# ShannonAI/GNN-LM

Hardware: AMD Instinct MI355X
Metric: eval tokens/sec on WikiText-103 (k=1024, GNN+KNN); test ppl match (higher is better)
Workload: dtype f32

## Files before the change

gnn-lm_amd/csrc/gemm_f32.hip:

```cpp
#include "kernels.h"

namespace gnnlm {

typedef float f32x16 __attribute__((ext_vector_type(16)));
typedef __bf16 bf16x8 __attribute__((ext_vector_type(8)));
typedef _Float16 f16x8 __attribute__((ext_vector_type(8)));

namespace {
constexpr int BK = 32, LDS_LD = BK + 4;
#ifndef GNNLM_GEMM_NBUF
#define GNNLM_GEMM_NBUF 1
#endif
constexpr int NBUF = GNNLM_GEMM_NBUF;
enum { EPI_STORE = 0, EPI_LSE = 1 };

__device__ __forceinline__ unsigned bf16_rn(float x) {
    const unsigned u = __float_as_uint(x);
    return (u + 0x7FFFu + ((u >> 16) & 1u)) >> 16;
}
__device__ __forceinline__ float bf16_to_f32(unsigned h) { return __uint_as_float(h << 16); }

template <int BM, int BN, int EPI, int NS>
__global__ __launch_bounds__(256, 3) void gemm_nt_f32_kernel(const GemmParams p) {
    constexpr int TM = BM / 64, TN = BN / 64;
    constexpr int LA = BM / 32, LW = BN / 32;
    constexpr int STAGE = (BM + BN) * LDS_LD;
    constexpr int SPLIT_LD = 20;
    constexpr int PLANE = (BM + BN) * SPLIT_LD;
    constexpr int LDS_FLOATS = NS == 0 ? NBUF * STAGE : NS * PLANE;
    __shared__ __attribute__((aligned(16))) float lds[LDS_FLOATS];

    const int tid = threadIdx.x, lane = tid & 63, wave = tid >> 6;
    const int wm = wave >> 1, wn = wave & 1;
    const int half = lane >> 5, l32 = lane & 31;

    int M = p.M;
    if (p.m_dev) M = min(M, *p.m_dev);
    if (p.m_out && blockIdx.x == 0 && threadIdx.x == 0) *p.m_out = M;
    const int tiles_n = (p.N + BN - 1) / BN;
    const int tiles_m = ((p.m_dev ? M : p.M) + BM - 1) / BM;
    const unsigned n_tiles = (unsigned)(tiles_m * tiles_n);
    const unsigned n_work = n_tiles * (unsigned)(p.batch1 * p.batch2);
    unsigned v = blockIdx.x;
    if (v >= n_work) return;

    const int kq = (tid & 7) * 4;
    const int srow = tid >> 3;
    const float* ap[LA];
    const float* wp[LW];
    float4 ra[LA], rw[LW];
    const int nk_full = p.K / BK;
    const bool k_tail = (p.K % BK) != 0;
    const float4 z4 = make_float4(0.f, 0.f, 0.f, 0.f);
    int m0x, n0x, b1x, b2x;

#define GNNLM_TILE_SETUP(w_)                                                                 \
    {                                                                                        \
        const unsigned by_ = (w_) / n_tiles, t = (w_) - by_ * n_tiles;                       \
        b1x = by_ / p.batch2; b2x = by_ % p.batch2;                                          \
        int tm, tn;                                                                          \
        if (p.tile_order == 1) { tm = t / tiles_n; tn = t % tiles_n; }                       \
        else if (p.tile_order == 2) { tn = t / tiles_m; tm = t % tiles_m; }                  \
        else {                   \
            const int GM = p.tile_order - 2;                                                 \
            const int band = t / (GM * tiles_n);                                             \
            const int m_in = min(GM, tiles_m - band * GM);                                   \
            const int r = t - band * GM * tiles_n;                                           \
            tn = r / m_in;                                                                   \
            tm = band * GM + r % m_in;                                                       \
        }                                                                                    \
        m0x = tm * BM; n0x = tn * BN;                                                        \
        const float* A_ = p.A + b1x * p.sA1 + b2x * p.sA2;                                   \
        const float* W_ = p.W + b1x * p.sW1 + b2x * p.sW2;                                   \
        _Pragma("unroll") for (int i = 0; i < LA; ++i) {                                     \
            const int gr = m0x + srow + 32 * i;                                              \
            int64_t ar = gr < M ? (p.a_rows ? (int64_t)p.a_rows[gr] : (int64_t)gr) : 0;      \
            if (ar < 0) ar = 0;       \
            ap[i] = A_ + ar * p.lda;                                                         \
        }                                                                                    \
        _Pragma("unroll") for (int i = 0; i < LW; ++i) {                                     \
            const int gn = n0x + srow + 32 * i;                                              \
            wp[i] = W_ + (int64_t)(gn < p.N ? gn : 0) * p.ldw;                               \
        }                                                                                    \
    }

#define GNNLM_LOAD_TILE(kt)                                                                  \
    {                                                                                        \
        const int k_ = (kt) * BK + kq;                                                       \
        _Pragma("unroll") for (int i_ = 0; i_ < LA; ++i_)                                    \
            ra[i_] = *reinterpret_cast<const float4*>(ap[i_] + k_);                          \
        _Pragma("unroll") for (int i_ = 0; i_ < LW; ++i_)                                    \
            rw[i_] = *reinterpret_cast<const float4*>(wp[i_] + k_);                          \
    }
#define GNNLM_LOAD_TILE_GUARDED(kt)                                                          \
    {                                                                                        \
        int k_ = (kt) * BK + kq;                                                             \
        const bool kin_ = k_ < p.K;                                                          \
        k_ = kin_ ? k_ : 0;                                                                  \
        _Pragma("unroll") for (int i_ = 0; i_ < LA; ++i_) {                                  \
            ra[i_] = *reinterpret_cast<const float4*>(ap[i_] + k_);                          \
            if (!kin_) ra[i_] = z4;                                                          \
        }                                                                                    \
        _Pragma("unroll") for (int i_ = 0; i_ < LW; ++i_) {                                  \
            rw[i_] = *reinterpret_cast<const float4*>(wp[i_] + k_);                          \
            if (!kin_) rw[i_] = z4;                                                          \
        }                                                                                    \
    }
#define GNNLM_PK_TRUNC(lo_, hi_) ((__float_as_uint(hi_) & 0xFFFF0000u) | (__float_as_uint(lo_) >> 16))
#define GNNLM_SPLIT_STORE(v_, row_)                                                          \
    {                                                                                        \
        char* dst_ = reinterpret_cast<char*>(lds) + (row_) * (SPLIT_LD * 4) + kq * 2;        \
        float r0_ = (v_).x, r1_ = (v_).y, r2_ = (v_).z, r3_ = (v_).w;                        \
        if constexpr (NS == 1) {                                                             \
            typedef _Float16 f16x4_ __attribute__((ext_vector_type(4)));                     \
            *reinterpret_cast<f16x4_*>(dst_) = f16x4_{(_Float16)r0_, (_Float16)r1_, (_Float16)r2_, (_Float16)r3_}; \
        } else if constexpr (NS == 3) {                                                             \
            _Pragma("unroll") for (int pl_ = 0; pl_ < 3; ++pl_) {                            \
                *reinterpret_cast<uint2*>(dst_ + pl_ * (PLANE * 4)) =                        \
                    make_uint2(GNNLM_PK_TRUNC(r0_, r1_), GNNLM_PK_TRUNC(r2_, r3_));          \
                r0_ -= __uint_as_float(__float_as_uint(r0_) & 0xFFFF0000u);                  \
                r1_ -= __uint_as_float(__float_as_uint(r1_) & 0xFFFF0000u);                  \
                r2_ -= __uint_as_float(__float_as_uint(r2_) & 0xFFFF0000u);                  \
                r3_ -= __uint_as_float(__float_as_uint(r3_) & 0xFFFF0000u);                  \
            }                                                                                \
        } else {                                                                             \
            _Pragma("unroll") for (int pl_ = 0; pl_ < 2; ++pl_) {                            \
                const unsigned b0_ = bf16_rn(r0_), b1_ = bf16_rn(r1_), b2_ = bf16_rn(r2_), b3_ = bf16_rn(r3_); \
                *reinterpret_cast<uint2*>(dst_ + pl_ * (PLANE * 4)) = make_uint2(b0_ | (b1_ << 16), b2_ | (b3_ << 16)); \
                r0_ -= __uint_as_float(b0_ << 16);                                           \
                r1_ -= __uint_as_float(b1_ << 16);                                           \
                r2_ -= __uint_as_float(b2_ << 16);                                           \
                r3_ -= __uint_as_float(b3_ << 16);                                           \
            }                                                                                \
        }                                                                                    \
    }
#define GNNLM_STORE_TILE(buf)                                                                \
    if constexpr (NS == 0) {                                                                 \
        float* a_ = &lds[(buf) * STAGE + srow * LDS_LD + kq];                                \
        float* w_ = a_ + BM * LDS_LD;                                                        \
        _Pragma("unroll") for (int i_ = 0; i_ < LA; ++i_)                                    \
            *reinterpret_cast<float4*>(a_ + 32 * i_ * LDS_LD) = ra[i_];                      \
        _Pragma("unroll") for (int i_ = 0; i_ < LW; ++i_)                                    \
            *reinterpret_cast<float4*>(w_ + 32 * i_ * LDS_LD) = rw[i_];                      \
    } else {                                                                                 \
        _Pragma("unroll") for (int i_ = 0; i_ < LA; ++i_) GNNLM_SPLIT_STORE(ra[i_], srow + 32 * i_)        \
        _Pragma("unroll") for (int i_ = 0; i_ < LW; ++i_) GNNLM_SPLIT_STORE(rw[i_], BM + srow + 32 * i_)   \
    }
#define GNNLM_SPLIT_MFMA(PA, PB)                                                             \
    _Pragma("unroll") for (int i = 0; i < TM; ++i)                                           \
        _Pragma("unroll") for (int j = 0; j < TN; ++j)                                       \
            acc[i][j] = EPI == EPI_LSE ? __builtin_amdgcn_mfma_f32_32x32x16_bf16(fb[PB][j], fa[PA][i], acc[i][j], 0, 0, 0)  \
                                       : __builtin_amdgcn_mfma_f32_32x32x16_bf16(fa[PA][i], fb[PB][j], acc[i][j], 0, 0, 0);
#define GNNLM_COMPUTE(buf)                                                                   \
    if constexpr (NS == 1) {                                                                 \
        const char* base_ = reinterpret_cast<const char*>(lds);                              \
        _Pragma("unroll") for (int ks_ = 0; ks_ < BK / 16; ++ks_) {                          \
            f16x8 ha[TM], hb[TN];                                                            \
            _Pragma("unroll") for (int i = 0; i < TM; ++i)                                   \
                ha[i] = *reinterpret_cast<const f16x8*>(base_ + (wm * (BM / 2) + 32 * i + l32) * SPLIT_LD * 4 + 32 * ks_ + 16 * half); \
            _Pragma("unroll") for (int j = 0; j < TN; ++j)                                   \
                hb[j] = *reinterpret_cast<const f16x8*>(base_ + (BM + wn * (BN / 2) + 32 * j + l32) * SPLIT_LD * 4 + 32 * ks_ + 16 * half); \
            _Pragma("unroll") for (int i = 0; i < TM; ++i)                                   \
                _Pragma("unroll") for (int j = 0; j < TN; ++j)                               \
                    acc[i][j] = EPI == EPI_LSE ? __builtin_amdgcn_mfma_f32_32x32x16_f16(hb[j], ha[i], acc[i][j], 0, 0, 0)  \
                                               : __builtin_amdgcn_mfma_f32_32x32x16_f16(ha[i], hb[j], acc[i][j], 0, 0, 0); \
        }                                                                                    \
    } else if constexpr (NS != 0) {                                                                 \
        const char* base_ = reinterpret_cast<const char*>(lds);                              \
        _Pragma("unroll") for (int ks_ = 0; ks_ < BK / 16; ++ks_) {                          \
            bf16x8 fa[NS][TM], fb[NS][TN];                                                   \
            _Pragma("unroll") for (int pl_ = 0; pl_ < NS; ++pl_) {                           \
                _Pragma("unroll") for (int i = 0; i < TM; ++i)                               \
                    fa[pl_][i] = *reinterpret_cast<const bf16x8*>(base_ + (pl_ * (BM + BN) + wm * (BM / 2) + 32 * i + l32) * SPLIT_LD * 4 + 32 * ks_ + 16 * half); \
                _Pragma("unroll") for (int j = 0; j < TN; ++j)                               \
                    fb[pl_][j] = *reinterpret_cast<const bf16x8*>(base_ + (pl_ * (BM + BN) + BM + wn * (BN / 2) + 32 * j + l32) * SPLIT_LD * 4 + 32 * ks_ + 16 * half); \
            }                                                                                \
            if constexpr (NS == 3) { GNNLM_SPLIT_MFMA(2, 0) GNNLM_SPLIT_MFMA(1, 1) GNNLM_SPLIT_MFMA(0, 2) }   \
            GNNLM_SPLIT_MFMA(1, 0) GNNLM_SPLIT_MFMA(0, 1) GNNLM_SPLIT_MFMA(0, 0)             \
        }                                                                                    \
    } else {                                                                                 \
        const float* a_base = &lds[(buf) * STAGE + (wm * (BM / 2) + l32) * LDS_LD + 4 * half];            \
        const float* w_base = &lds[(buf) * STAGE + (BM + wn * (BN / 2) + l32) * LDS_LD + 4 * half];       \
        _Pragma("unroll") for (int s_ = 0; s_ < BK / 8; ++s_) {                              \
            float4 a[TM], b[TN];                                                             \
            _Pragma("unroll") for (int i = 0; i < TM; ++i)                                   \
                a[i] = *reinterpret_cast<const float4*>(a_base + 32 * i * LDS_LD + 8 * s_);  \
            _Pragma("unroll") for (int j = 0; j < TN; ++j)                                   \
                b[j] = *reinterpret_cast<const float4*>(w_base + 32 * j * LDS_LD + 8 * s_);  \
            _Pragma("unroll") for (int i = 0; i < TM; ++i)                                   \
                _Pragma("unroll") for (int j = 0; j < TN; ++j) {                             \
                     \
                    if constexpr (EPI == EPI_LSE) {                                          \
                        acc[i][j] = __builtin_amdgcn_mfma_f32_32x32x2f32(b[j].x, a[i].x, acc[i][j], 0, 0, 0); \
                        acc[i][j] = __builtin_amdgcn_mfma_f32_32x32x2f32(b[j].y, a[i].y, acc[i][j], 0, 0, 0); \
                        acc[i][j] = __builtin_amdgcn_mfma_f32_32x32x2f32(b[j].z, a[i].z, acc[i][j], 0, 0, 0); \
                        acc[i][j] = __builtin_amdgcn_mfma_f32_32x32x2f32(b[j].w, a[i].w, acc[i][j], 0, 0, 0); \
                    } else {                                                                 \
                        acc[i][j] = __builtin_amdgcn_mfma_f32_32x32x2f32(a[i].x, b[j].x, acc[i][j], 0, 0, 0); \
                        acc[i][j] = __builtin_amdgcn_mfma_f32_32x32x2f32(a[i].y, b[j].y, acc[i][j], 0, 0, 0); \
                        acc[i][j] = __builtin_amdgcn_mfma_f32_32x32x2f32(a[i].z, b[j].z, acc[i][j], 0, 0, 0); \
                        acc[i][j] = __builtin_amdgcn_mfma_f32_32x32x2f32(a[i].w, b[j].w, acc[i][j], 0, 0, 0); \
                    }                                                                        \
                }                                                                            \
        }                                                                                    \
    }

#define GNNLM_LOAD_FIRST()                                                                   \
    if (nk_full > 0) GNNLM_LOAD_TILE(0) else GNNLM_LOAD_TILE_GUARDED(0)

    GNNLM_TILE_SETUP(xcd_remap(v, n_work))
    GNNLM_LOAD_FIRST()
    for (;;) {
        const int m0 = m0x, n0 = n0x, b1 = b1x, b2 = b2x;
        f32x16 acc[TM][TN];
#pragma unroll
        for (int i = 0; i < TM; ++i)
#pragma unroll
            for (int j = 0; j < TN; ++j)
#pragma unroll
                for (int r = 0; r < 16; ++r) acc[i][j][r] = 0.f;

        GNNLM_STORE_TILE(0);
        __syncthreads();
        if (nk_full > 0) {
            for (int kt = 0; kt < nk_full; ++kt) {
                constexpr bool ONE_BUF = NBUF == 1 || NS != 0;
                const int buf = ONE_BUF ? 0 : (kt & 1);
                if (kt + 1 < nk_full) GNNLM_LOAD_TILE(kt + 1);
                GNNLM_COMPUTE(buf);
                if (ONE_BUF) __syncthreads();
                if (kt + 1 < nk_full) { GNNLM_STORE_TILE(ONE_BUF ? 0 : (buf ^ 1)); }
                __syncthreads();
            }
            if (k_tail) {
                GNNLM_LOAD_TILE_GUARDED(nk_full);
                GNNLM_STORE_TILE(0);
                __syncthreads();
                GNNLM_COMPUTE(0);
                __syncthreads();
            }
        } else {
            GNNLM_COMPUTE(0);
            __syncthreads();
        }
        v += gridDim.x;
        const bool has_next = v < n_work;
        if (has_next) {
            GNNLM_TILE_SETUP(xcd_remap(v, n_work))
            GNNLM_LOAD_FIRST()
        }
        constexpr int WROWS = BM / 2, WCOLS = BN / 2;
#include "gemm_epilogue.inc"
        __syncthreads();
        if (!has_next) break;
    }
#undef GNNLM_LOAD_FIRST
#undef GNNLM_TILE_SETUP
#undef GNNLM_LOAD_TILE_GUARDED
#undef GNNLM_COMPUTE
#undef GNNLM_SPLIT_MFMA
#undef GNNLM_SPLIT_STORE
#undef GNNLM_PK_TRUNC
#undef GNNLM_LOAD_TILE
#undef GNNLM_STORE_TILE
}

template <int WPR>
__global__ __launch_bounds__(256) void lse_reduce_kernel(const float2* part, int n_parts, int64_t rows,
                                                         const int32_t* m_dev, float* lse) {
    __shared__ float2 red[4];
    const int lane = threadIdx.x & 63, wave = threadIdx.x >> 6;
    const int64_t row = WPR == 1 ? (int64_t)blockIdx.x * 4 + wave : (int64_t)blockIdx.x;
    if (row >= rows || (m_dev && row >= *m_dev)) return;
    const float2* pr = part + row * n_parts;
    const int i0 = WPR == 1 ? lane : threadIdx.x, step = 64 * WPR;
    float m = -INFINITY;
    for (int i = i0; i < n_parts; i += step) m = fmaxf(m, pr[i].x);
    m = wave_max(m);
    if (WPR == 4) {
        if (lane == 0) red[wave].x = m;
        __syncthreads();
        m = fmaxf(fmaxf(red[0].x, red[1].x), fmaxf(red[2].x, red[3].x));
    }
    float s = 0.f;
    for (int i = i0; i < n_parts; i += step) {
        const float2 v = pr[i];
        s += v.x == -INFINITY ? 0.f : v.y * expf(v.x - m);
    }
    s = wave_sum(s);
    if (WPR == 4) {
        if (lane == 0) red[wave].y = s;
        __syncthreads();
        s = (red[0].y + red[1].y) + (red[2].y + red[3].y);
    }
    if (threadIdx.x == (WPR == 1 ? 64 * wave : 0)) lse[row] = m + logf(s);
}

template <int BM, int BN, int NS>
void launch_ns(const GemmParams& p, dim3 grid, hipStream_t stream) {
    if constexpr (BN == 128) {
        if (p.lse_part) {
            hipLaunchKernelGGL((gemm_nt_f32_kernel<BM, BN, EPI_LSE, NS>), grid, dim3(256), 0, stream, p);
            return;
        }
    }
    hipLaunchKernelGGL((gemm_nt_f32_kernel<BM, BN, EPI_STORE, NS>), grid, dim3(256), 0, stream, p);
}
template <int BM, int BN>
void launch(const GemmParams& p, dim3 grid, hipStream_t stream) {
    if (p.precision == 1) launch_ns<BM, BN, 2>(p, grid, stream);
    else if (p.precision == 2) launch_ns<BM, BN, 3>(p, grid, stream);
    else if (p.precision == 3) launch_ns<BM, BN, 1>(p, grid, stream);
    else launch_ns<BM, BN, 0>(p, grid, stream);
}
}

thread_local int g_default_gemm_precision = 0;

int gemm_nt(const GemmParams& desc, hipStream_t stream) {
    GemmParams p = desc;
    if (p.precision == 0) p.precision = g_default_gemm_precision;
    if (p.alpha == 0.f) p.alpha = 1.f;
    if (p.batch1 == 0) p.batch1 = 1;
    if (p.batch2 == 0) p.batch2 = 1;
    GNNLM_REQUIRE(p.A && p.W && (p.C || p.lse_part), "gemm: null operand");
    GNNLM_REQUIRE(p.M >= 0 && p.N > 0 && p.K > 0, "gemm: bad shape");
    GNNLM_REQUIRE(p.K % 4 == 0 && p.lda % 4 == 0 && p.ldw % 4 == 0, "gemm: K, lda, ldw must be multiples of 4");
    GNNLM_REQUIRE(((uintptr_t)p.A % 16 == 0) && ((uintptr_t)p.W % 16 == 0), "gemm: operands must be 16-byte aligned");
    GNNLM_REQUIRE(p.sA1 % 4 == 0 && p.sA2 % 4 == 0 && p.sW1 % 4 == 0 && p.sW2 % 4 == 0, "gemm: batch strides must be multiples of 4");
    GNNLM_REQUIRE(p.batch1 >= 1 && p.batch2 >= 1, "gemm: bad batch");
    GNNLM_REQUIRE(p.precision >= 0 && p.precision <= 3, "gemm: precision must be 0 (f32 MFMA), 1 (bf16x3), 2 (bf16x6) or 3 (fp16)");
    GNNLM_REQUIRE(!p.lse_part || p.batch1 * p.batch2 == 1, "gemm: the LSE epilogue does not support batches");
    GNNLM_REQUIRE(!p.lse_part || p.alpha > 0.f, "gemm: the LSE epilogue needs alpha > 0");
    GNNLM_REQUIRE(!p.lse_part || (!p.bias && !p.gate && !p.R && !p.c_rows), "gemm: the LSE epilogue takes no bias, gate, R or c_rows");
    GNNLM_REQUIRE(p.tile_order >= 0 && p.tile_order <= 66, "gemm: tile_order must be 0 (auto), 1 (n fastest), 2 (m fastest) or 2+GM (bands of GM m-tiles)");
    if (p.M == 0) return OK;
    if (p.tile_order == 0)
        p.tile_order = (!p.m_dev && (double)p.M > (double)p.N) ? 1 : 2;
    if (gemm_split_eligible(p)) return gemm_nt_split(p, stream);
    if (gemm_skinny_eligible(p)) return gemm_nt_skinny(p, stream);
    const int64_t nb = (int64_t)p.batch1 * p.batch2;
    const int64_t tiles128 = cdiv(p.M, 128) * cdiv(p.N, 128) * nb;
    const bool small = !p.lse_part && tiles128 < 256;
    if (!small && gemm_sched_eligible(p)) return gemm_nt_sched(p, stream);
    if (!small && gemm_dma_eligible(p)) return gemm_nt_dma(p, stream);
    const int BMN = small ? 64 : 128;
    const int64_t tiles = cdiv(p.M, BMN) * cdiv(p.N, BMN) * nb;
    GNNLM_REQUIRE(tiles < (1ll << 31), "gemm: grid too large");
    const int64_t pool = 256 * (small ? 4 : (p.precision == 2 ? 2 : 3));
    dim3 grid((unsigned)std::min<int64_t>(tiles, pool));
    const double work = 2.0 * p.M * (double)p.N * p.K * nb;
    ProfScope prof(K_GEMM, stream, work, 4.0 * ((double)p.M * p.K + (double)p.N * p.K + (double)p.M * p.N) * nb,
                   p.m_dev, (double)p.M, true);
    if (prof.slot) p.m_out = prof.slot;
    if (small) launch<64, 64>(p, grid, stream);
    else launch<128, 128>(p, grid, stream);
    GNNLM_LAUNCH_CHECK();
    return OK;
}

int lse_reduce(const float* part, int n_parts, int64_t rows, const int32_t* m_dev, float* lse, hipStream_t stream) {
    GNNLM_REQUIRE(part && lse && n_parts > 0, "lse_reduce: bad arguments");
    if (rows == 0) return OK;
    ProfScope prof(K_LSE, stream, 0.0, 8.0 * rows * n_parts, m_dev, (double)rows);
    if (n_parts >= 1024)
        hipLaunchKernelGGL(lse_reduce_kernel<4>, dim3((unsigned)rows), dim3(256), 0, stream,
                           reinterpret_cast<const float2*>(part), n_parts, rows, m_dev, lse);
    else
        hipLaunchKernelGGL(lse_reduce_kernel<1>, dim3((unsigned)cdiv(rows, 4)), dim3(256), 0, stream,
                           reinterpret_cast<const float2*>(part), n_parts, rows, m_dev, lse);
    GNNLM_LAUNCH_CHECK();
    return OK;
}

}
```

gnn-lm_amd/csrc/kernels.h:

```cpp
#pragma once
#include "common.h"
#include "../../include/gnnlm.h"

namespace gnnlm {

typedef gnnlm_gemm_t GemmParams;
typedef gnnlm_gather_t GatherParams;
typedef gnnlm_star_attn_t StarAttnParams;
typedef gnnlm_chain_attn_t ChainAttnParams;
typedef gnnlm_knn_interp_t KnnInterpParams;
int topk_merge(const gnnlm_topk_t& d, hipStream_t stream);
int ivfpq_scan(const gnnlm_ivfpq_scan_t& d, hipStream_t stream);
int ivfpq_pack_codes(const uint8_t* codes, int64_t N, int M, uint8_t* out, hipStream_t stream);
int ivfpq_pack_lut(const float* lut, int64_t ld_lut, int64_t n, int M, float* out, hipStream_t stream);
int ivfpq_key_terms(const uint8_t* codes, const int64_t* list_off, int64_t N, int nlist, const float* coarse, const float* pq, int M, int dsub,
                    float* out, hipStream_t stream);

int ivfpq_pack_tiles(const uint8_t* codes, int64_t N, int M, uint8_t* out, hipStream_t stream);
int ivfpq_build_groups(const int64_t* pl, int64_t ld, int64_t n, int P, int nlist, int64_t seg, int32_t* grp_list, int32_t* grp_q,
                       int64_t* grp_out, int32_t* n_groups, int32_t* scratch, hipStream_t stream);
int ivfpq_quantize_lut(const float* lut, int64_t ld_lut, int64_t n, int M, uint8_t* qlut, float* qmeta, hipStream_t stream);
int ivfpq_scan8(const gnnlm_ivfpq_scan8_t& d, hipStream_t stream);
int ivfpq_rescore(const gnnlm_ivfpq_rescore_t& d, hipStream_t stream);
int ivfpq_tables(const gnnlm_ivfpq_tables_t& d, hipStream_t stream);
int ivfpq_split_payload(int64_t* idx, int64_t n, int label_bits, int32_t val_last, int32_t* out_vals, hipStream_t stream);
int ivfpq_tau(const gnnlm_ivfpq_tau_t& d, hipStream_t stream);
int ivfpq_select_probes(const gnnlm_ivfpq_select_probes_t& d, hipStream_t stream);
int ivfpq_select_final(const gnnlm_ivfpq_select_final_t& d, hipStream_t stream);

int gemm_nt(const GemmParams& p, hipStream_t stream);
bool gemm_split_eligible(const GemmParams& p);
int gemm_nt_split(const GemmParams& p, hipStream_t stream);
bool gemm_dma_eligible(const GemmParams& p);
int gemm_nt_dma(const GemmParams& p, hipStream_t stream);
bool gemm_sched_eligible(const GemmParams& p);
int gemm_nt_sched(const GemmParams& p, hipStream_t stream);
bool gemm_skinny_eligible(const GemmParams& p);
int gemm_nt_skinny(const GemmParams& p, hipStream_t stream);
extern thread_local int g_default_gemm_precision;
struct GemmPrecisionScope {
    int saved;
    explicit GemmPrecisionScope(int prec) : saved(g_default_gemm_precision) { g_default_gemm_precision = prec; }
    ~GemmPrecisionScope() { g_default_gemm_precision = saved; }
};
int lse_reduce(const float* part, int n_parts, int64_t rows, const int32_t* m_dev, float* lse, hipStream_t stream);
int gather_decode(const GatherParams& p, hipStream_t stream);
int pq_encode(const float* x, int64_t ldx, const float* cen, const float* norm2, int M, int dsub, int64_t n, uint8_t* codes,
              hipStream_t stream);
int token_gather(const gnnlm_token_gather_t& p, hipStream_t stream);
int neighbor_labels(const int64_t* ids, int64_t n, int64_t n_store, const void* vals, int itemsize, int n_vocab, int32_t* out,
                    hipStream_t stream);
int bucket_rows(const int64_t* rows, int64_t n, int64_t n_store, int64_t per, int world, int self, int64_t* counts,
                int64_t* cursor, int64_t* send_rows, int32_t* inv, hipStream_t stream);
int gather_rows_peer(const gnnlm_peer_gather_t& d, hipStream_t stream);
int bucket_rows_padded(const int64_t* rows, int64_t n, int64_t n_store, int64_t per, int world, int64_t cap, int64_t* cursor,
                       int64_t* send_rows, int32_t* inv, int64_t* overflow, hipStream_t stream);
int star_attn(const StarAttnParams& p, hipStream_t stream);
bool star_attn_tab_eligible(const StarAttnParams& p);
int star_attn_tab(const StarAttnParams& p, hipStream_t stream);

__device__ __forceinline__ const uint8_t* shard_row_ptr(const gnnlm_shards_t* sh, int64_t row, int M) {
    const int64_t per = sh->rows_per_rank;
    const int64_t q = ((uint64_t)(row | per) >> 32) == 0 ? (int64_t)((uint32_t)row / (uint32_t)per) : row / per;
    const int g = (int)min((int64_t)sh->n - 1, q);
    const int64_t local = row - sh->row0[g];
    return local >= 0 && local < sh->rows[g] ? sh->base[g] + local * M : nullptr;
}
__device__ __forceinline__ int64_t star_group(const StarAttnParams& p, int i, int j) {
    const int64_t e = (int64_t)i * p.kg + j;
    return p.x_index ? (int64_t)p.x_index[e] : e;
}
__device__ __forceinline__ bool star_nb_ok(const StarAttnParams& p, int i, int j, int64_t id) {
    bool ok = id >= 0 && (p.n_store <= 0 || id < p.n_store);
    if (p.shards) ok = ok && shard_row_ptr(p.shards, id, p.M) != nullptr;
    else if (p.codes && !p.codes_direct) ok = ok && id - p.row0 >= 0 && id - p.row0 < p.n_local;
    if (ok && (p.nb_valid || p.x_index)) {
        const int64_t gi = star_group(p, i, j);
        ok = gi >= 0 && (!p.nb_valid || p.nb_valid[gi * p.nb_valid_stride] != 0);
    }
    return ok;
}
__device__ __forceinline__ int64_t star_code_row(const StarAttnParams& p, int i, int j, int64_t id) {
    if (!p.codes_direct) return id - p.row0;
    const int64_t s = ((int64_t)i * p.kg + j) * p.codes_direct;
    return p.codes_index ? (int64_t)p.codes_index[s] : s;
}
__device__ __forceinline__ const uint8_t* star_code_ptr(const StarAttnParams& p, int i, int j, int64_t id) {
    if (p.shards) return shard_row_ptr(p.shards, id, p.M);
    return p.codes + star_code_row(p, i, j, id) * p.M;
}
bool star_attn_dense_eligible(const StarAttnParams& p);
int star_attn_dense(const StarAttnParams& p, hipStream_t stream);
int chain_attn(const ChainAttnParams& p, hipStream_t stream);

int causal_softmax(float* S, int64_t n_mats, int T, int64_t ld, int max_ctx, hipStream_t stream);
bool causal_attn_fused_ok(int T, int dk);
int causal_attn_fused(const float* Q, const float* K, const float* V, int64_t ld, float* out, int64_t ldo,
                      int n_blocks, int T, int H, int dk, int max_ctx, hipStream_t stream, bool accumulate = false);

bool causal_attn_varlen_ok(int dk);
int causal_attn_varlen(const float* Q, const float* K, const float* V, int64_t ld, float* out, int64_t ldo, const gnnlm_ragged_t& rg,
                       int H, int dk, int max_ctx, hipStream_t stream, bool accumulate = false);
bool decode_attn_ok(int dk);
int check_kv_cache(const gnnlm_kv_cache_t& c);
size_t decode_attn_workspace_bytes(int B, int H, int dk, int max_len);
struct SlotTable { const int32_t* src; int64_t ld; };
int decode_attn(const gnnlm_decode_attn_t& d, const SlotTable* tab, hipStream_t stream);
int beam_select(const gnnlm_beam_select_t& d, hipStream_t stream);
int kv_cache_fill(const float* qkv, int64_t ld_src, const gnnlm_kv_cache_t& c, int layer, const gnnlm_ragged_t& rg, int max_rows,
                  hipStream_t stream);
int kv_len_set(const gnnlm_kv_cache_t& c, const int32_t* block_off, int max_rows, hipStream_t stream);
int kv_len_advance(const gnnlm_kv_cache_t& c, int bound, hipStream_t stream);
int sample_topk(const gnnlm_sample_topk_t& d, hipStream_t stream);
int64_t ragged_tiles(const int32_t* block_off, int n_blocks, int32_t* tiles);

int layernorm(const float* x, int64_t ldx, const float* gamma, const float* beta, float* out, int64_t ldo,
              int64_t rows, int d, float eps, const uint8_t* valid, hipStream_t stream,
              const float* residual = nullptr, int64_t ldr = 0,
              const int32_t* rows_idx = nullptr,
              const int32_t* n_dev = nullptr, int n_mult = 1);
int group_rows(int32_t* idx, int64_t n_groups, int n_g, const int* sel, int n_sel, hipStream_t stream);
int scatter_rows(const float* src, int64_t ld_src, float* dst, int64_t ld_dst, const int32_t* slots, int64_t n, int d, hipStream_t stream,
                 const int32_t* n_dev = nullptr);

int group_assign(const gnnlm_group_assign_t& d, hipStream_t stream);
int slot_rows(const int64_t* centres, int64_t G, const int32_t* n_dev, int left, int right, int reach, int64_t n_store, int64_t* out, hipStream_t stream);
int window_counts(const int32_t* n_dev, int64_t cap, int64_t per, int n_win, int32_t* counts, hipStream_t stream);
int nb_code_rows(const int32_t* group_index, const int32_t* fetched_index, int n_g, int64_t n, int32_t* out, hipStream_t stream);
int scatter_code_rows(const uint8_t* src, const int32_t* index, int64_t stride, const uint8_t* valid, uint8_t* dst, const int32_t* slots,
                      const int32_t* n_dev, int64_t cap, int bytes, hipStream_t stream);

int mean2(const float* a, const float* b, float* out, int64_t n, hipStream_t stream);

int gelu(float* x, int64_t n, hipStream_t stream);
int relu(float* x, int64_t n, hipStream_t stream);

int filter_neighbors(const int64_t* ids, const int64_t* pos, int64_t n, int kg, int64_t ctx, int64_t* out, hipStream_t stream);

int half_to_float(const void* src, float* dst, int64_t n, hipStream_t stream);

int row_lse_pick(const float* logits, int64_t ld, int64_t rows, const int32_t* m_dev, int n,
                 const int32_t* pick, float* lse, float* picked, hipStream_t stream);

struct BandSplitParams {
    const int64_t* target = nullptr; int64_t n = 0;
    int n_bands = 0; int32_t cutoff[8] = {0};
    int32_t* head_pick = nullptr;
    int32_t* band_rows = nullptr;
    int32_t* band_pick = nullptr;
    int32_t* band_count = nullptr;
};
int band_split(const BandSplitParams& p, hipStream_t stream);

int head_logp(const float* picked, const float* lse, const int32_t* pick, float* out, int64_t n, hipStream_t stream);
int tail_combine(const float* tail_picked, const float* tail_lse, const int32_t* rows,
                 const int32_t* count_dev, int64_t n_max, float* lm_logp, hipStream_t stream);

int knn_interp(const KnnInterpParams& p, hipStream_t stream);
int label_tags(const void* vals, int itemsize, int64_t n, uint8_t* tag, hipStream_t stream);
size_t knn_interp_scratch_bytes(int64_t n, int k, int64_t n_local);
bool knn_interp_bucketed_eligible(const KnnInterpParams& p);
int knn_interp_bucketed(const KnnInterpParams& p, float log_1ml, float log_l, hipStream_t stream);
int knn_interp_grid(const gnnlm_knn_interp_grid_t& d, int n_lm, int64_t ld_lm, hipStream_t stream);
int logp_mix(const float* gnn_logp, const float* base_logp, int64_t n, const double* alphas, int n_alphas, float* out, hipStream_t stream);
int knn_recompute_sims(const gnnlm_knn_resim_t& d, hipStream_t stream);

int masked_sum_f64(const float* x, const uint8_t* mask, int64_t n, double* out, hipStream_t stream);
int rows_sum_f64(const float* x, int64_t ld, int64_t rows, int64_t n, double* out, hipStream_t stream);

}
```

Before: 569,700.

## Add short-K f32 GEMM path with register-resident A and overlapped stores

Adds a dedicated f32 MFMA GEMM kernel for K ≤ 256 (multiple of 32). Each block holds its 128-row A slice in registers, streams 64-column W tiles through double-buffered LDS, and walks across N. In the plain case it ping-pongs two accumulator sets so the buffer stores of the previous tile's C overlap the MFMAs of the current tile. This targets short-K projections that are bound by C writes and launch shape in the generic kernel. The cost is extra registers and LDS, plus another dispatch branch with its own alignment conditions.

```diff
diff --git a/gnn-lm_amd/csrc/gemm_f32.hip b/gnn-lm_amd/csrc/gemm_f32.hip
--- a/gnn-lm_amd/csrc/gemm_f32.hip
+++ b/gnn-lm_amd/csrc/gemm_f32.hip
@@ -339,6 +339,7 @@
         p.tile_order = (!p.m_dev && (double)p.M > (double)p.N) ? 1 : 2;
     if (gemm_split_eligible(p)) return gemm_nt_split(p, stream);
     if (gemm_skinny_eligible(p)) return gemm_nt_skinny(p, stream);
+    if (gemm_shortk_eligible(p)) return gemm_nt_shortk(p, stream);
     const int64_t nb = (int64_t)p.batch1 * p.batch2;
     const int64_t tiles128 = cdiv(p.M, 128) * cdiv(p.N, 128) * nb;
     const bool small = !p.lse_part && tiles128 < 256;
diff --git a/gnn-lm_amd/csrc/gemm_f32_shortk.hip b/gnn-lm_amd/csrc/gemm_f32_shortk.hip
--- /dev/null
+++ b/gnn-lm_amd/csrc/gemm_f32_shortk.hip
@@ -0,0 +1,241 @@
+#include "kernels.h"
+
+#include <stdlib.h>
+
+namespace gnnlm {
+
+typedef float f32x16 __attribute__((ext_vector_type(16)));
+typedef float f32x4 __attribute__((ext_vector_type(4)));
+
+namespace {
+enum { EPI_STORE = 0, EPI_LSE = 1 };
+#ifndef GNNLM_SK_EXP
+#define GNNLM_SK_EXP 0
+#endif
+
+template <int NKT, bool PLAIN>
+__global__ __launch_bounds__(256, NKT <= 4 ? 2 : 1) void gemm_nt_f32_shortk_kernel(const GemmParams p, const int nslots) {
+    constexpr int EPI = EPI_STORE;
+    constexpr int K = 32 * NKT, KG = K / 8;
+    constexpr int BM = 128, BN = 64, TM = 1, TN = 2, WROWS = 32, WCOLS = 64;
+    constexpr int TILE = BN * K;
+    constexpr int NW = 2 * NKT;
+    constexpr int KGS = GNNLM_SK_EXP == 3 ? 0 : (KG >= 4 ? KG * 3 / 4 : KG);
+    extern __shared__ __attribute__((aligned(16))) float wt[];
+    float* lds = wt;
+
+    const int tid = threadIdx.x, lane = tid & 63;
+    const int wave = __builtin_amdgcn_readfirstlane(tid >> 6);
+    const int wm = wave, wn = 0;
+    const int half = lane >> 5, l32 = lane & 31;
+
+    int M = p.M;
+    if (p.m_dev) M = min(M, *p.m_dev);
+    if (p.m_out && blockIdx.x == 0 && threadIdx.x == 0) *p.m_out = M;
+    const int tiles_n = (p.N + BN - 1) / BN;
+    const int tiles_m = (M + BM - 1) / BM;
+    const unsigned n_work = (unsigned)(tiles_m * p.batch1 * p.batch2) * (unsigned)nslots;
+    const unsigned ldc4 = (unsigned)p.ldc * 4u;
+
+    int rd[4];
+#pragma unroll
+    for (int s = 0; s < 4; ++s) rd[s] = l32 * 32 + 4 * ((2 * s + half) ^ ((l32 >> 1) & 7));
+    const int srow = tid >> 3, chunk = tid & 7;
+    const int sw0 = srow * 32 + 4 * (chunk ^ ((srow >> 1) & 7));
+
+    for (unsigned w = blockIdx.x; w < n_work; w += gridDim.x) {
+        const unsigned unit = w / (unsigned)nslots;
+        const int slot = (int)(w - unit * (unsigned)nslots);
+        const int by = (int)(unit / (unsigned)tiles_m), tm = (int)(unit - (unsigned)by * (unsigned)tiles_m);
+        const int b1 = by / p.batch2, b2 = by % p.batch2;
+        const int m0 = tm * BM;
+        const float* Wb = p.W + b1 * p.sW1 + b2 * p.sW2;
+
+        float4 areg[KG];
+        {
+            const int gr = m0 + wave * WROWS + l32;
+            int64_t ar = gr < M ? (p.a_rows ? (int64_t)p.a_rows[gr] : (int64_t)gr) : 0;
+            if (ar < 0) ar = 0;
+            const float* arow = p.A + b1 * p.sA1 + b2 * p.sA2 + ar * p.lda + 4 * half;
+#pragma unroll
+            for (int s = 0; s < KG; ++s) areg[s] = *reinterpret_cast<const float4*>(arow + 8 * s);
+        }
+#define GNNLM_SK_LOAD_W(nt_)                                                                 \
+    {                                                                                        \
+        const int g0_ = (nt_) * BN + srow, g1_ = g0_ + 32;                                   \
+        const float* w0_ = Wb + (int64_t)(g0_ < p.N ? g0_ : 0) * p.ldw + 4 * chunk;          \
+        const float* w1_ = Wb + (int64_t)(g1_ < p.N ? g1_ : 0) * p.ldw + 4 * chunk;          \
+        _Pragma("unroll") for (int kt = 0; kt < NKT; ++kt) {                                 \
+            rw[2 * kt] = *reinterpret_cast<const f32x4*>(w0_ + 32 * kt);                    \
+            rw[2 * kt + 1] = *reinterpret_cast<const f32x4*>(w1_ + 32 * kt);                \
+        }                                                                                    \
+    }
+#define GNNLM_SK_PUT_W(buf_)                                                                 \
+    _Pragma("unroll") for (int kt = 0; kt < NKT; ++kt) {                                     \
+        *reinterpret_cast<f32x4*>(wt + (buf_) * TILE + kt * (BN * 32) + sw0) = rw[2 * kt];  \
+        *reinterpret_cast<f32x4*>(wt + (buf_) * TILE + kt * (BN * 32) + 1024 + sw0) = rw[2 * kt + 1]; \
+    }
+#define GNNLM_SK_STORE(PREV, t_)                                                             \
+    {                                                                                        \
+        const int j_ = (t_) >> 4, r_ = (t_) & 15, ro_ = (r_ & 3) + 8 * (r_ >> 2);            \
+        __builtin_amdgcn_raw_buffer_store_b32(__float_as_uint(PREV[j_][r_] * p.alpha), crs,  \
+                                              (int)((GNNLM_SK_EXP == 1 ? 0x80000000u : vprev[j_]) + (unsigned)ro_ * (GNNLM_SK_EXP == 4 ? 0u : ldc4)), 0, 0); \
+    }
+#define GNNLM_SK_TILE(ACC, PREV, HAVE_PREV)                                                  \
+    {                                                                                        \
+        const float* sb_ = wt + buf * TILE;                                                  \
+        _Pragma("unroll") for (int j = 0; j < TN; ++j)                                       \
+            _Pragma("unroll") for (int r = 0; r < 16; ++r) ACC[j][r] = 0.f;                  \
+        float4 b_[2][TN];                                                                    \
+        _Pragma("unroll") for (int j = 0; j < TN; ++j)                                       \
+            b_[0][j] = *reinterpret_cast<const float4*>(sb_ + j * 1024 + rd[0]);             \
+        _Pragma("unroll") for (int s = 0; s < KG; ++s) {                                     \
+            if (s + 1 < KG) {                                                                \
+                _Pragma("unroll") for (int j = 0; j < TN; ++j)                               \
+                    b_[(s + 1) & 1][j] = *reinterpret_cast<const float4*>(sb_ + ((s + 1) >> 2) * (BN * 32) + j * 1024 + rd[(s + 1) & 3]); \
+            }                                                                                \
+            _Pragma("unroll") for (int j = 0; j < TN; ++j) {                                 \
+                ACC[j] = __builtin_amdgcn_mfma_f32_32x32x2f32(areg[s].x, b_[s & 1][j].x, ACC[j], 0, 0, 0); \
+                ACC[j] = __builtin_amdgcn_mfma_f32_32x32x2f32(areg[s].y, b_[s & 1][j].y, ACC[j], 0, 0, 0); \
+                ACC[j] = __builtin_amdgcn_mfma_f32_32x32x2f32(areg[s].z, b_[s & 1][j].z, ACC[j], 0, 0, 0); \
+                ACC[j] = __builtin_amdgcn_mfma_f32_32x32x2f32(areg[s].w, b_[s & 1][j].w, ACC[j], 0, 0, 0); \
+            }                                                                                \
+            if (HAVE_PREV && s < KGS) {                                                      \
+                _Pragma("unroll") for (int t = 0; t < 32; ++t)                               \
+                    if (t >= s * 32 / (KGS ? KGS : 1) && t < (s + 1) * 32 / (KGS ? KGS : 1)) GNNLM_SK_STORE(PREV, t) \
+            }                                                                                \
+            __builtin_amdgcn_sched_barrier(0);       \
+        }                                                                                    \
+        if (GNNLM_SK_EXP == 3 && HAVE_PREV) {                                                \
+            _Pragma("unroll") for (int t = 0; t < 32; ++t) GNNLM_SK_STORE(PREV, t)           \
+        }                                                                                    \
+    }
+
+        int nt = slot;
+        int buf = 0;
+        {
+            f32x4 rw[NW];
+            GNNLM_SK_LOAD_W(nt)
+            GNNLM_SK_PUT_W(0)
+        }
+        __builtin_amdgcn_s_waitcnt(0x0F70);
+        __syncthreads();
+        if constexpr (PLAIN) {
+            const int rowbase = m0 + wave * WROWS + 4 * half;
+            const uint64_t cb = (uint64_t)(uintptr_t)(p.C + b1 * p.sC1 + b2 * p.sC2);
+            const __amdgpu_buffer_rsrc_t crs = __builtin_amdgcn_make_buffer_rsrc(
+                (void*)(uintptr_t)(((uint64_t)(uint32_t)__builtin_amdgcn_readfirstlane((int)(uint32_t)(cb >> 32)) << 32) |
+                                   (uint32_t)__builtin_amdgcn_readfirstlane((int)(uint32_t)cb)),
+                0, (int)((unsigned)M * ldc4), 0x00020000);
+            const unsigned vrow = (unsigned)rowbase * ldc4 + 4u * (unsigned)l32;
+            unsigned vprev[TN] = {0x80000000u, 0x80000000u};
+            f32x16 acc0[TN], acc1[TN];
+            for (;;) {
+                f32x4 rw[NW];
+                const bool more0 = nt + nslots < tiles_n;
+                if (more0 && GNNLM_SK_EXP != 2) GNNLM_SK_LOAD_W(nt + nslots)
+                GNNLM_SK_TILE(acc0, acc1, true)
+#pragma unroll
+                for (int j = 0; j < TN; ++j) vprev[j] = nt * BN + 32 * j + l32 < p.N ? vrow + 4u * (unsigned)(nt * BN + 32 * j) : 0x80000000u;
+                if (!more0) {
+#pragma unroll
+                    for (int t = 0; t < 32; ++t) GNNLM_SK_STORE(acc0, t)
+                    break;
+                }
+                if (GNNLM_SK_EXP != 2) { GNNLM_SK_PUT_W(buf ^ 1) buf ^= 1; }
+                nt += nslots;
+                __syncthreads();
+                const bool more1 = nt + nslots < tiles_n;
+                if (more1 && GNNLM_SK_EXP != 2) GNNLM_SK_LOAD_W(nt + nslots)
+                GNNLM_SK_TILE(acc1, acc0, true)
+#pragma unroll
+                for (int j = 0; j < TN; ++j) vprev[j] = nt * BN + 32 * j + l32 < p.N ? vrow + 4u * (unsigned)(nt * BN + 32 * j) : 0x80000000u;
+                if (!more1) {
+#pragma unroll
+                    for (int t = 0; t < 32; ++t) GNNLM_SK_STORE(acc1, t)
+                    break;
+                }
+                if (GNNLM_SK_EXP != 2) { GNNLM_SK_PUT_W(buf ^ 1) buf ^= 1; }
+                nt += nslots;
+                __syncthreads();
+            }
+        } else {
+            for (;;) {
+                f32x4 rw[NW];
+                const int n0 = nt * BN;
+                const bool more = nt + nslots < tiles_n;
+                if (more) GNNLM_SK_LOAD_W(nt + nslots)
+                f32x16 acc[TM][TN];
+                {
+                    const __amdgpu_buffer_rsrc_t crs = __builtin_amdgcn_make_buffer_rsrc((void*)nullptr, 0, 0, 0x00020000);
+                    const unsigned vprev[TN] = {0x80000000u, 0x80000000u};
+                    GNNLM_SK_TILE(acc[0], acc[0], false)
+                }
+#include "gemm_epilogue.inc"
+                if (!more) break;
+                if (GNNLM_SK_EXP != 2) { GNNLM_SK_PUT_W(buf ^ 1) buf ^= 1; }
+                nt += nslots;
+                __syncthreads();
+            }
+        }
+        __syncthreads();
+#undef GNNLM_SK_TILE
+#undef GNNLM_SK_STORE
+#undef GNNLM_SK_PUT_W
+#undef GNNLM_SK_LOAD_W
+    }
+}
+
+template <int NKT>
+int launch_shortk(const GemmParams& p, int nslots, dim3 grid, hipStream_t stream) {
+    constexpr size_t lds_bytes = 2 * (size_t)(64 * 32 * NKT) * sizeof(float);
+    if (!p.bias && !p.R && !p.c_rows && !p.a_rows) {
+        GNNLM_LDS_OPT_IN((&gemm_nt_f32_shortk_kernel<NKT, true>), lds_bytes);
+        hipLaunchKernelGGL((gemm_nt_f32_shortk_kernel<NKT, true>), grid, dim3(256), lds_bytes, stream, p, nslots);
+    } else {
+        GNNLM_LDS_OPT_IN((&gemm_nt_f32_shortk_kernel<NKT, false>), lds_bytes);
+        hipLaunchKernelGGL((gemm_nt_f32_shortk_kernel<NKT, false>), grid, dim3(256), lds_bytes, stream, p, nslots);
+    }
+    return OK;
+}
+}
+
+bool gemm_shortk_eligible(const GemmParams& p) {
+    const char* e = getenv("GNNLM_GEMM_SHORTK");
+    if (e && atoi(e) == 0) return false;
+    if (p.precision != 0 || p.lse_part) return false;
+    if (p.K % 32 != 0 || p.K > 256) return false;
+    if ((uintptr_t)p.C % 128 != 0 || p.ldc % 32 != 0 || p.sC1 % 32 != 0 || p.sC2 % 32 != 0) return false;
+    if (p.ldc < p.N || ((int64_t)p.M + 128) * p.ldc * 4 >= (1ll << 31)) return false;
+    return true;
+}
+
+int gemm_nt_shortk(const GemmParams& p_in, hipStream_t stream) {
+    GemmParams p = p_in;
+    const int64_t nb = (int64_t)p.batch1 * p.batch2;
+    const int64_t units = cdiv(p.M, 128) * nb, tiles_n = cdiv(p.N, 64);
+    GNNLM_REQUIRE(units * tiles_n < (1ll << 31), "gemm: grid too large");
+    const int64_t pool = 512;
+    const int nslots = (int)std::max<int64_t>(1, std::min<int64_t>(tiles_n, pool / units));
+    dim3 grid((unsigned)std::min<int64_t>(units * nslots, pool));
+    const double work = 2.0 * p.M * (double)p.N * p.K * nb;
+    ProfScope prof(K_GEMM, stream, work, 4.0 * ((double)p.M * p.K + (double)p.N * p.K + (double)p.M * p.N) * nb,
+                   p.m_dev, (double)p.M, true);
+    if (prof.slot) p.m_out = prof.slot;
+    int rc;
+    switch (p.K / 32) {
+        case 1: rc = launch_shortk<1>(p, nslots, grid, stream); break;
+        case 2: rc = launch_shortk<2>(p, nslots, grid, stream); break;
+        case 3: rc = launch_shortk<3>(p, nslots, grid, stream); break;
+        case 4: rc = launch_shortk<4>(p, nslots, grid, stream); break;
+        case 5: rc = launch_shortk<5>(p, nslots, grid, stream); break;
+        case 6: rc = launch_shortk<6>(p, nslots, grid, stream); break;
+        case 7: rc = launch_shortk<7>(p, nslots, grid, stream); break;
+        default: rc = launch_shortk<8>(p, nslots, grid, stream); break;
+    }
+    if (rc != OK) return rc;
+    GNNLM_LAUNCH_CHECK();
+    return OK;
+}
+
+}
diff --git a/gnn-lm_amd/csrc/kernels.h b/gnn-lm_amd/csrc/kernels.h
--- a/gnn-lm_amd/csrc/kernels.h
+++ b/gnn-lm_amd/csrc/kernels.h
@@ -37,6 +37,8 @@
 int gemm_nt_sched(const GemmParams& p, hipStream_t stream);
 bool gemm_skinny_eligible(const GemmParams& p);
 int gemm_nt_skinny(const GemmParams& p, hipStream_t stream);
+bool gemm_shortk_eligible(const GemmParams& p);
+int gemm_nt_shortk(const GemmParams& p, hipStream_t stream);
 extern thread_local int g_default_gemm_precision;
 struct GemmPrecisionScope {
     int saved;
```

After: 572,000 (median of 6 runs). About the same (+0.4%).
